# LuchnikovI/Differentiable-quantum-circuit-cuda

Hardware: AMD Instinct MI355X
Metric: gate-applications/sec (fwd+bwd) at n qubits (higher is better)
Workload: dtype c64 (f32)

## Files before the change

differentiable-quantum-circuit-cuda_amd/csrc/qdc.hip:

```cpp
#include "qdc_circuit.hpp"
#include "qdc_primitives.hpp"
#include "qdc_spec.hpp"

namespace {
template <int R>
struct SpecCheckTwo {
  __device__ __forceinline__ void operator()(qdc::cx (&xf)[R], qdc::cx (&xb)[R], const qdc::SpecEnv& E) const {
    constexpr uint32_t z[32] = {};
    qdc::spec_xchg_imm<6, false>(xf, E, z, z);
    qdc::spec_xchg<6, false>(xb, E, z, z, z, z);
  }
};
template <int R, int TB>
struct SpecCheckOne {
  __device__ __forceinline__ void operator()(qdc::cx (&x)[R], const qdc::SpecEnv& E) const {
    constexpr uint32_t z[32] = {};
    qdc::spec_xchg_imm<TB, true>(x, E, z, z);
    qdc::spec_xchg<TB, true>(x, E, z, z, z, z);
  }
};
}
#define QDC_SPEC_CHECK(name, threads, pass)                                                       \
  __global__ __launch_bounds__(threads) void name(qdc::chunk* f, qdc::chunk* b, const qdc::fop* ops, \
                                                  const qdc::cx* mats, qdc::fgeo fg, uint32_t l0,    \
// ... 354 lines not shown
    }
    x.prof.on = on != 0;
  }
  return nullptr;
}

QDC_API size_t qdc_circuit_profile_collect(qdc_circuit* c, qdc_kernel_stat* out, size_t cap) {
  std::vector<qdc::Ctx*> xs;
  for (auto& d : c->impl.devs) xs.push_back(&d->ctx);
  return qdc::prof_collect(xs, out, cap);
}

QDC_API size_t qdc_circuit_host_times(qdc_circuit* c, double* out, size_t n, int reset) {
  size_t k = 0;
  for (int d = 0; d < 2; ++d)
    for (int j = 0; j < 6; ++j, ++k)
      if (out && k < n) out[k] = c->impl.host_ms[d][j];
  if (reset)
    for (auto& row : c->impl.host_ms)
      for (double& v : row) v = 0;
  return std::min<size_t>(n, 12);
}

QDC_API const char* qdc_build_info(void) {
#ifdef QDC_F64
  return "qdc f64 gfx950";
#else
  return "qdc f32 gfx950";
#endif
}

QDC_API size_t qdc_fusion_schedule(size_t local_qubits, int backward, size_t first_inject,
                                   const int* kinds, const unsigned char* inexact,
                                   size_t n_instr, const qdc_plan_op* plan, size_t n_plan,
                                   int lcmin, int max_ops, unsigned* item_info, size_t item_cap,
                                   unsigned* stage_len, size_t stage_cap, unsigned* op_order,
                                   size_t op_cap) {
  std::vector<qdc::Instr> ins(n_instr);
  for (size_t k = 0; k < n_instr; ++k) ins[k] = qdc::Instr{kinds[k], 0, 0};
  std::vector<uint8_t> sens(n_instr, 0);
  if (inexact)
    for (size_t k = 0; k < n_instr; ++k) sens[k] = inexact[k] ? 1 : 0;
  qdc::FusionPlanner P{ins, sens, (uint32_t)local_qubits, true, true,
                             max_ops > 0 ? (uint32_t)std::min(max_ops, qdc::FMAX_OPS)
                                         : (uint32_t)qdc::FMAX_OPS,
                             lcmin > 0 ? (uint32_t)lcmin : 3u};
  using qdc::Knob;
  P.tile2_chunks = qdc::knob_uint(Knob::TILE2_CHUNKS, P.tile2_chunks);
  P.tile1_chunks = qdc::knob_uint(Knob::TILE1_CHUNKS, P.tile1_chunks);
  P.permute = P.rq_grad = qdc::knob_int(Knob::SCHED_RQ, 0) != 0;
  P.permute = qdc::knob_int(Knob::SCHED_PERM, P.permute) != 0;
  P.mirror = qdc::knob_int(Knob::SCHED_MIRROR, P.mirror) != 0;
  P.defer_q1 = qdc::knob_int(Knob::DEFER_Q1, P.defer_q1) != 0;
  P.perm_low = qdc::knob_uint(Knob::RQ_PERM_LOW, P.perm_low);
  P.gamma_stage_cap = qdc::knob_int(Knob::RQ_GSTAGE, P.gamma_stage_cap) != 0;
  P.split_dens = qdc::knob_int(Knob::DENS_SPLIT, P.split_dens) != 0;
  std::vector<qdc_plan_op> pl(plan, plan + n_plan);
  const std::vector<qdc::FusionItem> items = P.fuse_items(pl, backward != 0, first_inject);
  size_t ns = 0, no = 0;
  for (size_t i = 0; i < items.size(); ++i) {
    const qdc::FusionItem& it = items[i];
    std::vector<std::vector<uint32_t>> stages;
    if (it.type == 2)
      stages = P.stage_partition(it.ops, pl, backward != 0);
    else
      stages.push_back(it.ops);
    if (i >= item_cap || ns + stages.size() > stage_cap) return SIZE_MAX;
    unsigned* info = item_info + 12 * i;
    info[0] = (unsigned)it.type;
    info[1] = (unsigned)stages.size();
    info[2] = it.lc;
    info[3] = it.h;
    for (int k = 0; k < 8; ++k) info[4 + k] = k < (int)qdc::FMAX_ROWS ? it.hb[k] : 0u;
    for (const auto& st : stages) {
      stage_len[ns++] = (unsigned)st.size();
      for (uint32_t op : st) {
        if (no >= op_cap) return SIZE_MAX;
        op_order[no++] = op;
      }
    }
  }
  return items.size();
}

QDC_API int qdc_gate_plan(unsigned n, unsigned R, unsigned pos2, unsigned pos1,
                          int two_states, int far_tile, unsigned* out) {
  if (!out || (R != 2 && R != 4) || n < 2 || n > 62 || pos2 >= n || pos1 >= n ||
      (R == 2 && pos2 != pos1) || (R == 4 && pos2 == pos1))
    return -1;
  const qdc::Plan p = qdc::plan_gate(n, (int)R, pos2, pos1, two_states != 0, 1024u, far_tile != 0);
  const uint64_t cnt = p.tile ? p.tg.ntiles : p.g.items;
  const unsigned v[10] = {p.tile ? 1u : 0u, (unsigned)p.mode, p.tg.l, p.tg.h, p.tg.hb0, p.tg.hb1,
                          p.tg.t1, p.tg.t2, (unsigned)(cnt & 0xffffffffu), (unsigned)(cnt >> 32)};
  for (int i = 0; i < 10; ++i) out[i] = v[i];
  return 0;
}

QDC_API int qdc_lane_plan(unsigned n, unsigned R, unsigned pos2, unsigned pos1, int reduces,
                          unsigned* out) {
  if (!out || (R != 2 && R != 4) || n < 2 || n > 62 || pos2 >= n || pos1 >= n ||
      (R == 2 && pos2 != pos1) || (R == 4 && pos2 == pos1))
    return -1;
  qdc::Plan p;
  if (!qdc::plan_lane(n, (int)R, pos2, pos1, 2048u, (reduces & 1) != 0, p, 1, (reduces & 2) ? 10u : 6u))
    return 1;
  const qdc::lgeo& g = p.lg;
// ... 305 lines not shown
```

differentiable-quantum-circuit-cuda_amd/csrc/qdc_circuit.hpp:

```cpp
#pragma once

#include <algorithm>
#include <cstring>
#include <memory>
#include <vector>

#include <rccl/rccl.h>

#include "qdc/circuit.h"
#include "qdc_device.hpp"
#include "qdc_shard.hpp"
#include "qdc_stage.hpp"
#include "qdc_fusion.hpp"
#include "qdc_jit.hpp"

namespace qdc {

struct Flat {
  const qdc_complex* data;
  std::vector<size_t> off;
  std::vector<size_t> len;
  Flat(const qdc_complex* d, const size_t* lens, size_t n) : data(d), off(n), len(n) {
    size_t o = 0;
    for (size_t i = 0; i < n; ++i) {
// ... 162 lines not shown
    return nullptr;
  }
  void destroy() {
    for (auto e : ev) (void)hipEventDestroy(e);
    ev.clear();
    for (auto c : comms) (void)ncclCommDestroy(c);
    comms.clear();
  }
};

struct Circuit {
  uint32_t n = 0;
  uint32_t g = 0;
  uint32_t nl = 0;
  uint32_t gap_bits = 0;
  uint64_t gm = 0;
  std::vector<std::unique_ptr<DevRes>> devs;
  Exchange ex;
  std::vector<Shard> sh;
  QubitMap layout;
  size_t dens_cap = 0, grads_cap = 0;
  cx* host_out = nullptr;
  size_t host_cap = 0;
  std::vector<Instr> ins;
  struct Knobs {
    int fuse = 1;
    uint32_t fuse_max_ops = FMAX_OPS;
    uint32_t fuse_lcmin = 3;
    int fuse_meas = 1;
    int use_rq = 1;
    int rq_stats = 0;
    RqKnobs rqk;
    int rq64 = 1;
    int rq_order = 2;
    int spec_mode = 1;
    uint32_t spec_min_qubits = 22;
    uint32_t spec_max = 160;
    int spec_fwd = 1;
    int spec_async = sizeof(real) == 4 ? 1 : 0;
    int rq_permute = 1;
    int rq_perm_shard = 1;
    int rq_grad32 = 1;
    int rq_maxcl = 1;
    uint32_t rq_perm_low = 0;
    int rq_gstage = 1;
    uint32_t tile1_chunks = FusionPlanner::TILE_CHUNKS_1;
    int diag_inject = 1;
    int early_inject = 1;
    int dens1_kernel = 1;
    int dens_split = 1;
    int mirror = 1;
    int spec_half = 1;
    int defer_q1 = 1;
    uint32_t fused_blocks = 0;
    int sched_cache_on = 1;
    int state_ilv = 1;
    uint32_t state_ilv_bits = 12;

    template <class K, class F>
    static void each(K& k, F&& f) {
      f(Knob::FUSE, k.fuse);
      f(Knob::FUSE_MAX_OPS, k.fuse_max_ops, 1, FMAX_OPS);
      f(Knob::FUSE_MEAS, k.fuse_meas);
      f(Knob::FUSE_LCMIN, k.fuse_lcmin, 1, LOWBITS);
      f(Knob::FUSED_BLOCKS, k.fused_blocks, 1, (int)NBMAX);
      f(Knob::RQ, k.use_rq);
      f(Knob::RQ64, k.rq64);
      f(Knob::RQ_STATS, k.rq_stats);
      f(Knob::RW, k.rqk.rq_wave);
      f(Knob::RQ_PF, k.rqk.rq_prefetch);
      f(Knob::RQ_SLOTS5, k.rqk.rq_slots5);
      f(Knob::RQ_ORDER, k.rq_order);
      f(Knob::RQ_PERM, k.rq_permute);
      f(Knob::RQ_PERM_SHARD, k.rq_perm_shard);
      f(Knob::RQ_PERM_LOW, k.rq_perm_low);
      f(Knob::RQ_GRAD32, k.rq_grad32);
      f(Knob::RQ_MAXCL, k.rq_maxcl);
      f(Knob::RQ_GSTAGE, k.rq_gstage);
      f(Knob::TILE1_CHUNKS, k.tile1_chunks);
      f(Knob::DIAG_INJECT, k.diag_inject);
      f(Knob::EARLY_INJECT, k.early_inject);
      f(Knob::DENS1, k.dens1_kernel);
      f(Knob::DENS_SPLIT, k.dens_split);
      f(Knob::MIRROR, k.mirror);
      f(Knob::DEFER_Q1, k.defer_q1);
      f(Knob::SCHED_CACHE, k.sched_cache_on);
      f(Knob::SPEC, k.spec_mode);
      f(Knob::SPEC_MIN_QUBITS, k.spec_min_qubits);
      f(Knob::SPEC_MAX, k.spec_max);
      f(Knob::SPEC_FWD, k.spec_fwd);
      f(Knob::SPEC_ASYNC, k.spec_async);
      f(Knob::SPEC_HALF, k.spec_half);
      f(Knob::STATE_ILV, k.state_ilv);
      f(Knob::STATE_ILV_BITS, k.state_ilv_bits, 4, 24);
    }
    const char* read() {
      each(*this, KnobRead{});
      constexpr uint32_t T1 = FusionPlanner::TILE_CHUNKS_1, T2 = FusionPlanner::TILE_CHUNKS_2;
      if (tile1_chunks != T1 && tile1_chunks != T2)
        return fail("%s must be %u or %u", KNOB_TABLE[(int)Knob::TILE1_CHUNKS].name, T1, T2);
      return nullptr;
    }
  } k;
  double host_ms[2][6] = {};
  using hclock = std::chrono::steady_clock;
  static double ms_between(hclock::time_point a, hclock::time_point b) {
    return std::chrono::duration<double, std::milli>(b - a).count();
  }
  void host_record(int dir, const hclock::time_point (&t)[6]) {
    host_ms[dir][0] += 1;
    for (int k = 1; k < 6; ++k) host_ms[dir][k] += ms_between(t[k - 1], t[k]);
  }
  std::map<std::vector<uint32_t>, SpecEntry> spec_cache;
  uint64_t spec_epoch = 0;
  bool mirror_on() const {
    return k.mirror && k.fuse && k.fuse_max_ops >= 2 && k.use_rq && (sizeof(real) == 4 || k.rq64);
  }
  const char* rq_variant(bool two, uint32_t tbits, const RqVariant*& V) const {
    V = rq_select(two, tbits, k.rqk, mirror_on());
    if (!V)
      return fail("no register-resident kernel for a %u-amplitude %s tile", 1u << tbits,
                  two ? "two-state" : "one-state");
    return nullptr;
  }
  bool rq_keep(const RqVariant& V) const { return k.spec_half && V.ns == 5; }

  bool dry = false;
  std::vector<unsigned char> dry_prog;
  std::vector<SpecEntry*> dry_specs;
  struct TraceOp {
    uint32_t dir, item, q2, q1, R, diag, mirrored, single;
    qdc_complex m[16];
  };
  bool tracing = false;
  std::vector<TraceOp> trace;
  size_t trace_from = 0;
  std::vector<uint8_t> inexact;
  std::vector<std::pair<const void*, uint32_t>> fused_resident_cache;
// ... 428 lines not shown
      size_t ng = f.stages.size();
      while (ng > 0 && is_meas(mrec.plan[f.stages[ng - 1][0]])) --ng;
      for (size_t j = ng; j < f.stages.size(); ++j)
        for (uint32_t fi : f.stages[j])
          if (!is_meas(mrec.plan[fi])) return false;
      if (ng < f.stages.size()) {
        Item m = shell();
        for (size_t j = f.stages.size(); j-- > ng;) {
          const uint32_t bi = push(f.stages[j][0]);
          m.ops.push_back(bi);
          m.stages.push_back({bi});
        }
        if (m.ops.size() == 1) {
          m.type = 0;
          m.stages.clear();
        }
        items.push_back(std::move(m));
      }
      if (ng == 0) continue;
      Item b = shell();
      for (auto it = f.swaps.rbegin(); it != f.swaps.rend(); ++it) b.swaps.push_back(*it);
      for (size_t j = ng; j-- > 0;) {
        std::vector<uint32_t> st;
        for (size_t t = f.stages[j].size(); t-- > 0;) {
          if (is_meas(mrec.plan[f.stages[j][t]])) return false;
          const uint32_t bi = push(f.stages[j][t]);
          st.push_back(bi);
          b.ops.push_back(bi);
        }
        b.stages.push_back(std::move(st));
        b.mirror_of.push_back({(uint32_t)k, (uint32_t)j});
      }
      items.push_back(std::move(b));
    }
    first_inject = first_injection(pl);
    return true;
  }
  size_t first_injection(const std::vector<qdc_plan_op>& pl) const {
    for (size_t i = 0; i < pl.size(); ++i)
      if (pl[i].type == QDC_PLAN_OP && is_diff_density(ins[pl[i].instr].kind)) return i;
    return pl.size();
  }
  static constexpr uint32_t TILE_CHUNKS_1 = FusionPlanner::TILE_CHUNKS_1;
  static constexpr uint32_t TILE_CHUNKS_2 = FusionPlanner::TILE_CHUNKS_2;
  FusionPlanner planner() const {
    FusionPlanner P{ins, inexact, nl, k.fuse != 0, k.fuse_meas != 0, k.fuse_max_ops, k.fuse_lcmin};
    P.permute = k.rq_permute && k.use_rq && (g == 0 || k.rq_perm_shard) && sizeof(real) == 4;
    P.ng = g;
    P.rq_grad = k.rq_grad32 && k.use_rq && (sizeof(real) == 4 || k.rq64);
    if (k.rq_perm_low) P.perm_low = k.rq_perm_low;
    P.tile1_chunks = k.tile1_chunks;
    P.mirror = mirror_on() && sched_mirror;
    P.defer_q1 = k.defer_q1 != 0;
    P.gamma_stage_cap = k.rq_gstage != 0;
    P.split_dens = k.dens_split != 0;
    return P;
  }
  bool is_meas(const qdc_plan_op& op) const { return planner().is_meas(op); }
  std::vector<Item> fuse_items(std::vector<qdc_plan_op>& plan, bool backward,
                               size_t first_inject = SIZE_MAX) const {
    std::vector<Item> items;
    for (FusionItem& f : planner().fuse_items(plan, backward, first_inject)) {
      Item it;
      static_cast<FusionItem&>(it) = std::move(f);
      if (it.type == 2) it.stages = planner().stage_partition(it.ops, plan, backward);
      items.push_back(std::move(it));
    }
    return items;
  }
  struct SchedCache {
    bool valid = false;
    size_t first_inject = 0;
    bool mirror = false;
    std::vector<qdc_plan_op> in_plan, out_plan;
    std::vector<uint8_t> inexact;
    std::vector<Item> items;
  };
  SchedCache sched_cache[2];
  bool sched_mirror = false;
  static bool same_plan(const std::vector<qdc_plan_op>& a, const std::vector<qdc_plan_op>& b) {
    if (a.size() != b.size()) return false;
    for (size_t i = 0; i < a.size(); ++i) {
      const qdc_plan_op &x = a[i], &y = b[i];
      if (x.type != y.type || x.instr != y.instr || x.pos2 != y.pos2 || x.pos1 != y.pos1 ||
          x.nvictims != y.nvictims || x.pack != y.pack)
        return false;
      for (unsigned k = 0; k < x.nvictims && k < 8; ++k)
        if (x.victims[k] != y.victims[k]) return false;
    }
    return true;
  }
  std::vector<Item> schedule(std::vector<qdc_plan_op>& plan, bool backward, size_t first_inject) {
    SchedCache& c = sched_cache[backward ? 1 : 0];
    if (k.sched_cache_on && c.valid && c.first_inject == first_inject && c.inexact == inexact &&
        c.mirror == sched_mirror && same_plan(c.in_plan, plan)) {
      plan = c.out_plan;
      return c.items;
    }
    c.valid = false;
    c.in_plan = plan;
    std::vector<Item> items = fuse_items(plan, backward, first_inject);
    if (k.sched_cache_on) {
      c.out_plan = plan;
      c.items = items;
      c.inexact = inexact;
      c.first_inject = first_inject;
// ... 1036 lines not shown
```

differentiable-quantum-circuit-cuda_amd/csrc/qdc_fusion.hpp:

```cpp
#pragma once

#include <stdint.h>

#include <algorithm>
#include <vector>

#include "qdc/circuit.h"
#include "qdc_kernels.hpp"
#include "qdc_knobs.hpp"
#include "qdc_rq.hpp"
#include "qdc_shard.hpp"

namespace qdc {

struct Instr {
  int kind;
  uint32_t a;
  uint32_t b;
};

inline bool is_q1_gate(int k) {
  return k == QDC_CONST_Q1 || k == QDC_CONST_Q1_NONU || k == QDC_VAR_Q1 || k == QDC_VAR_Q1_NONU;
}
inline bool is_q2_dense(int k) {
  return k == QDC_CONST_Q2 || k == QDC_VAR_Q2 || k == QDC_CONST_Q2_NONU || k == QDC_VAR_Q2_NONU;
}
inline bool is_diag(int k) { return k == QDC_CONST_Q2_DIAG || k == QDC_VAR_Q2_DIAG; }
inline bool is_const(int k) {
  return k == QDC_CONST_Q1 || k == QDC_CONST_Q1_NONU || k == QDC_CONST_Q2 ||
         k == QDC_CONST_Q2_NONU || k == QDC_CONST_Q2_DIAG;
}
inline bool is_var(int k) {
  return k == QDC_VAR_Q1 || k == QDC_VAR_Q1_NONU || k == QDC_VAR_Q2 || k == QDC_VAR_Q2_NONU ||
         k == QDC_VAR_Q2_DIAG;
}
inline bool is_nonu(int k) {
  return k == QDC_CONST_Q1_NONU || k == QDC_VAR_Q1_NONU || k == QDC_CONST_Q2_NONU ||
         k == QDC_VAR_Q2_NONU;
}
inline bool is_density(int k) {
  return k == QDC_Q1_DENSITY || k == QDC_Q2_DENSITY || k == QDC_DIFF_Q1_DENSITY ||
         k == QDC_DIFF_Q2_DENSITY;
}
inline bool is_diff_density(int k) {
  return k == QDC_DIFF_Q1_DENSITY || k == QDC_DIFF_Q2_DENSITY;
}
inline bool is_q1_density(int k) { return k == QDC_Q1_DENSITY || k == QDC_DIFF_Q1_DENSITY; }
inline int gate_len(int k) { return is_q2_dense(k) ? 16 : 4; }

struct FusionItem {
  int type;
  std::vector<uint32_t> ops;
  uint32_t lc = 0, h = 0, hb[FMAX_ROWS] = {};
  std::vector<std::pair<uint32_t, uint32_t>> swaps;
};

struct FusionPlanner {
  static constexpr uint32_t TILE_CHUNKS_1 = 2048;
  static constexpr uint32_t TILE_CHUNKS_2 = 1024;
  const std::vector<Instr>& ins;
  const std::vector<uint8_t>& inexact;
  uint32_t nl;
  bool fuse;
  bool fuse_meas;
  uint32_t fuse_max_ops;
  uint32_t fuse_lcmin;
  uint32_t tile2_chunks = TILE_CHUNKS_2;
  uint32_t tile1_chunks = TILE_CHUNKS_1;
  bool permute = false;
  bool rq_grad = false;
  bool gamma_stage_cap = true;
  uint32_t perm_low = (uint32_t)LV + 3;
  uint32_t ng = 0;
  bool mirror = false;
  bool defer_q1 = true;
  bool split_dens = true;

  static uint32_t log2_of(uint64_t x) {
    uint32_t k = 0;
    while ((1ull << k) < x) ++k;
    return k;
  }

  uint64_t chunk_bits_of(uint32_t p) const { return p >= (uint32_t)LV ? 1ull << (p - LV) : 0ull; }
  bool tile_config(uint64_t mask, uint32_t T, uint32_t& lc, uint32_t& h, uint32_t* hb) const {
    const uint32_t cbits = nl - LV;
    if (cbits < T) return false;
    for (int l = (int)T; l >= (int)fuse_lcmin; --l) {
      uint32_t rows = 0, tmp[64];
      for (uint32_t c = (uint32_t)l; c < cbits; ++c)
        if (mask >> c & 1ull) tmp[rows++] = c;
      if (rows > (uint32_t)FMAX_ROWS || (uint32_t)l + rows > T) continue;
      for (uint32_t c = (uint32_t)l; c < cbits && (uint32_t)l + rows < T; ++c)
        if (!(mask >> c & 1ull)) tmp[rows++] = c;
      if ((uint32_t)l + rows != T || rows > (uint32_t)FMAX_ROWS) continue;
      std::sort(tmp, tmp + rows);
      lc = (uint32_t)l;
      h = rows;
      for (uint32_t k = 0; k < rows; ++k) hb[k] = tmp[k];
      return true;
    }
    return false;
  }
  bool tile_fits(uint64_t mask, uint32_t T) const {
    if (nl - LV < T) return false;
    for (int l = (int)T; l >= (int)fuse_lcmin; --l) {
      const uint32_t rows = (uint32_t)__builtin_popcountll(mask >> l);
      if (rows <= (uint32_t)FMAX_ROWS && (uint32_t)l + rows <= T) return true;
    }
    return false;
  }

  bool is_meas(const qdc_plan_op& op) const {
    return op.type == QDC_PLAN_OP && is_density(ins[op.instr].kind);
  }
  uint32_t op_class(const qdc_plan_op& op, bool backward) const {
    if (op.type != QDC_PLAN_OP) return 0;
    const bool inex = op.instr < inexact.size() && inexact[op.instr];
    if (mirror && !backward)
      return order_class(ins[op.instr].kind, false, inex) | order_class(ins[op.instr].kind, true, inex);
    return order_class(ins[op.instr].kind, backward, inex);
  }
  static uint32_t conflicts_of(uint32_t c) { return order_conflicts(c); }
  bool is_gate_op(const qdc_plan_op& op) const {
    if (op.type != QDC_PLAN_OP) return false;
    const int k = ins[op.instr].kind;
    return is_const(k) || is_var(k);
  }
  uint64_t op_bits(const qdc_plan_op& op) const {
// ... 77 lines not shown
    remap_map(nv, mn);
    for (uint32_t p = 0; p < nl + ng; ++p) mvi[mv[p]] = p;
    for (uint32_t x = 0; x < nl + ng; ++x) out[x] = mn[pi[mvi[x]]];
    pi.swap(out);
    r.pack = 0;
    for (uint32_t j = 0; j < ng; ++j) {
      r.victims[j] = nv[j];
      r.pack |= (nv[j] != nl - ng + j) ? 1 : 0;
    }
  }

  std::vector<FusionItem> fuse_items(std::vector<qdc_plan_op>& plan, bool backward,
                                     size_t first_inject = SIZE_MAX) const {
    std::vector<FusionItem> items;
    const bool mfwd = mirror && !backward;
    const uint32_t T = log2_of((backward || mfwd) ? tile2_chunks : tile1_chunks);
    const bool on = fuse && fuse_max_ops >= 2;
    size_t msplit = SIZE_MAX;
    if (mfwd)
      for (size_t k = plan.size(); k-- > 0;)
        if (plan[k].type == QDC_PLAN_OP && is_meas(plan[k]) &&
            (ins[plan[k].instr].kind == QDC_DIFF_Q1_DENSITY ||
             ins[plan[k].instr].kind == QDC_DIFF_Q2_DENSITY)) {
          msplit = k + 1;
          break;
        }
    auto fusable = [&](size_t k) {
      const qdc_plan_op& op = plan[k];
      if (!(is_gate_op(op) || (fuse_meas && is_meas(op))) || !tile_fits(op_bits(op), T))
        return false;
      return !(backward && is_meas(op) && k < first_inject);
    };
    size_t i = 0;
    while (i < plan.size()) {
      const qdc_plan_op& op = plan[i];
      if (op.type == QDC_PLAN_REMAP) {
        items.push_back(FusionItem{1, {(uint32_t)i}});
        ++i;
        continue;
      }
      if (!on || !fusable(i)) {
        items.push_back(FusionItem{0, {(uint32_t)i}});
        ++i;
        continue;
      }
      size_t j = i;
      while (j < plan.size() && plan[j].type == QDC_PLAN_OP && fusable(j) &&
             !(backward && j == first_inject && j > i) && !(j == msplit && j > i))
        ++j;
      const bool two = (backward && i >= first_inject) || mfwd;
      const bool gstage = two && rq_grad && gamma_stage_cap;
      const uint32_t gmax = gstage ? fuse_max_ops
                            : (two && rq_grad) ? (uint32_t)FMAX_GRAD_RQ : (uint32_t)FMAX_GRAD;
      std::vector<uint32_t> rem;
      for (size_t k = i; k < j; ++k) rem.push_back((uint32_t)k);
      while (!rem.empty()) {
        uint64_t mask = 0, blocked = 0;
        uint32_t nred = 0;
        uint32_t ndens = 0;
        uint32_t left = 0;
        std::vector<uint32_t> pass, rest;
        int kind = -1;
        for (uint32_t k : rem) {
          const qdc_plan_op& g = plan[k];
          const uint64_t q = (1ull << g.pos2) | (1ull << g.pos1);
          const bool meas = is_meas(g);
          const uint32_t cls = op_class(g, backward);
          const uint32_t isred = mfwd ? (is_var(ins[g.instr].kind) ? 1u : 0u)
                                 : ((!backward && meas) || (two && is_var(ins[g.instr].kind))) ? 1u : 0u;
          if ((backward && kind >= 0 && (int)meas != kind) || (mfwd && kind == 1 && !meas) ||
              (!backward && split_dens && kind == 0 && meas) ||
              (q & blocked) ||
              (mfwd && meas && ndens + 1 > (uint32_t)FMAX_GRAD) ||
              (conflicts_of(cls) & left) || pass.size() >= fuse_max_ops ||
              nred + isred > gmax || !tile_fits(mask | op_bits(g), T)) {
            blocked |= q;
            left |= cls;
            rest.push_back(k);
            continue;
          }
          pass.push_back(k);
          mask |= op_bits(g);
          nred += isred;
          ndens += (mfwd && meas) ? 1u : 0u;
          kind = (int)meas;
        }
        if (gstage && nred > (uint32_t)FMAX_GRAD_RQ) {
          bool cut = false;
          while (pass.size() > 1 && gamma_stages(pass, plan, !mfwd) > (uint32_t)FMAX_GRAD_RQ) {
            rest.push_back(pass.back());
            pass.pop_back();
            cut = true;
          }
          if (cut) {
            std::sort(rest.begin(), rest.end());
            mask = 0;
            for (uint32_t k : pass) mask |= op_bits(plan[k]);
          }
        }
        if (defer_q1 && defer_trailing_q1(pass, rest, plan, backward)) {
          mask = 0;
          for (uint32_t k : pass) mask |= op_bits(plan[k]);
        }
        if (pass.size() == 1) {
          items.push_back(FusionItem{0, pass});
        } else {
          FusionItem it{2, pass};
          tile_config(mask, T, it.lc, it.h, it.hb);
          bool gates_only = it.lc >= NLOW - LV;
          for (uint32_t k : pass) gates_only = gates_only && is_gate_op(plan[k]);
          if (permute && gates_only) permute_after(it, plan, rest, j);
          items.push_back(it);
        }
        rem.swap(rest);
      }
      i = j;
    }
    return items;
  }

  bool defer_trailing_q1(std::vector<uint32_t>& pass, std::vector<uint32_t>& rest,
                         const std::vector<qdc_plan_op>& plan, bool backward) const {
    if (pass.size() < 2 || rest.empty()) return false;
    const std::vector<std::vector<uint32_t>> sts = stage_partition(pass, plan, backward);
    if (sts.size() < 2) return false;
    std::vector<uint32_t> moved;
    size_t kept_stages = sts.size();
    for (const auto& st : sts) {
      if (kept_stages <= 1) break;
      bool q1only = true;
      for (uint32_t k : st)
        q1only = q1only && is_gate_op(plan[k]) && plan[k].pos2 == plan[k].pos1 &&
                 plan[k].pos2 == plan[st[0]].pos2;
      if (!q1only) continue;
      const uint32_t qb = plan[st[0]].pos2;
      const uint64_t qm = 1ull << qb;
      bool free = true;
      for (uint32_t x : st) {
        const uint32_t cx = op_class(plan[x], backward);
        for (uint32_t y : pass) {
          if (y <= x || std::find(st.begin(), st.end(), y) != st.end()) continue;
          if (std::find(moved.begin(), moved.end(), y) != moved.end()) continue;
          const uint64_t yq = (1ull << plan[y].pos2) | (1ull << plan[y].pos1);
          if ((yq & qm) || (conflicts_of(cx) & op_class(plan[y], backward))) free = false;
        }
      }
      if (!free) continue;
      const qdc_plan_op* next = nullptr;
      for (uint32_t k : rest)
        if (k > st.back() && (((1ull << plan[k].pos2) | (1ull << plan[k].pos1)) & qm)) {
          next = &plan[k];
          break;
        }
      if (!next || !is_gate_op(*next) || next->pos2 == next->pos1) continue;
      moved.insert(moved.end(), st.begin(), st.end());
      --kept_stages;
    }
    if (moved.empty()) return false;
    std::vector<uint32_t> keep;
    for (uint32_t k : pass)
      if (std::find(moved.begin(), moved.end(), k) == moved.end()) keep.push_back(k);
    pass.swap(keep);
    rest.insert(rest.end(), moved.begin(), moved.end());
    std::sort(rest.begin(), rest.end());
    return true;
  }

  uint32_t gamma_stages(const std::vector<uint32_t>& pass, const std::vector<qdc_plan_op>& plan,
                        bool backward = true) const {
    uint32_t n = 0;
    for (const auto& st : stage_partition(pass, plan, backward)) {
      bool var = false;
      for (uint32_t k : st) var = var || (plan[k].type == QDC_PLAN_OP && is_var(ins[plan[k].instr].kind));
      n += var ? 1u : 0u;
    }
    return n;
  }

  std::vector<std::vector<uint32_t>> stage_partition(const std::vector<uint32_t>& pass,
                                                     const std::vector<qdc_plan_op>& plan,
                                                     bool backward) const {
    std::vector<std::vector<uint32_t>> stages;
    std::vector<uint32_t> rem = pass;
    while (!rem.empty()) {
      std::vector<uint32_t> st, rest;
      uint64_t q = 0, blocked = 0;
      uint32_t left = 0;
      bool closed = false;
      for (uint32_t k : rem) {
        if (closed) {
          rest.push_back(k);
          continue;
        }
        const qdc_plan_op& g = plan[k];
        const uint64_t gq = (1ull << g.pos2) | (1ull << g.pos1);
        const bool meas = is_meas(g);
        const uint32_t cls = op_class(g, backward);
        bool bad = (gq & blocked) || (conflicts_of(cls) & left);
        if (!bad && meas) {
          if (st.empty()) {
            st.push_back(k);
            closed = true;
            continue;
          }
          bad = true;
        }
        if (!bad && __builtin_popcountll(q | gq) > 2) bad = true;
        if (bad) {
          blocked |= gq;
          left |= cls;
          rest.push_back(k);
          continue;
        }
        st.push_back(k);
        q |= gq;
      }
      stages.push_back(std::move(st));
      rem.swap(rest);
    }
    return stages;
  }

};

struct RqStage {
  uint32_t kind, t1, t2;
  uint64_t deps = 0;
};
constexpr int RQ_SLOTS_MAX = 5;
struct RqLayout {
  uint32_t ns = 4;
  uint32_t slot[RQ_SLOTS_MAX] = {~0u, ~0u, ~0u, ~0u, ~0u};
  bool tfix = false;
  uint32_t tfirst[3] = {0, 0, 0};
  static RqLayout empty(uint32_t ns) {
    RqLayout L;
    L.ns = ns;
    return L;
  }
  bool operator==(const RqLayout& o) const {
    if (ns != o.ns || tfix != o.tfix) return false;
    for (uint32_t s = 0; s < ns; ++s)
      if (slot[s] != o.slot[s]) return false;
    return !tfix || (tfirst[0] == o.tfirst[0] && tfirst[1] == o.tfirst[1] &&
                     tfirst[2] == o.tfirst[2]);
  }
  uint32_t threads(uint32_t T, uint32_t* out) const {
    uint32_t k = 0;
    if (tfix)
      for (int i = 0; i < 3; ++i) out[k++] = tfirst[i];
    for (uint32_t q = 0; q < T && k < 8; ++q) {
      if (holds(q)) continue;
      if (tfix && (q == tfirst[0] || q == tfirst[1] || q == tfirst[2])) continue;
      out[k++] = q;
    }
    return k;
  }
  int find(uint32_t q) const {
    for (uint32_t s = 0; s < ns; ++s)
      if (slot[s] == q) return (int)s;
// ... 256 lines not shown
```

differentiable-quantum-circuit-cuda_amd/csrc/qdc_knobs.hpp:

```cpp
#pragma once

#include <stdint.h>

#include <algorithm>
#include <climits>
#include <cstdio>
#include <cstdlib>
#include <string>

namespace qdc {

enum class KnobScope { Process, Context, Circuit, Call, Hook };

#define QDC_KNOBS(X)                                                                               \
                                                        \
  X(DYN, Context, "35",                                                                            \
    "static share (% of the fair share) of a dynamic-tail pass; 100: static only")                 \
  X(DYN_GRAN, Context, "1",                                                                        \
    "smallest granule (tiles per grab, a power of two <= 32) of a reducing dynamic tail")          \
  X(EVENT_FENCE, Context, "0",                                                                     \
    "1: the profiler's HIP events are default events (system-scope fence per record)")             \
  X(GRID_CAP, Context, "1048576", "grid cap of the single-gate streaming kernels")                 \
  X(RED_CAP, Context, "2048", "grid of the single-gate reduction kernels (<= 4096)")               \
  X(REV_RED, Context, "4096",                                                                      \
// ... 7 lines not shown
  X(TILE2_WIDE, Context, "2", "two-state tile-family launches on 2^(9 + w)-chunk tiles")           \
  X(TILE1_WIDE, Context, "2", "one-state tile-family launches on 2^(10 + w)-chunk tiles")          \
  X(LANE, Context, "2",                                                                            \
    "single-gate ops on the LANE family, bits: 1 reverse, 2 streaming one-state, 4 densities "     \
    "/ gradients")                                                                                 \
  X(DIAG_RU, Context, "16",                                                                        \
    "chunks per state in flight per thread of the diagonal reverse kernels")                       \
  X(DIAG_Q, Context, "1", "0: diagonal reverse launches on k_diag instead of k_diag_q")            \
  X(DIAG_RED, Context, "4096", "grid of the diagonal reverse's reducing launches (<= 4096)")       \
  X(TILE_PF, Context, "1", "0: tile-family blocks of several tiles do not prefetch the next tile") \
  X(LANE_BLK, Context, "1",                                                                        \
    "0: far-target streaming LANE launches stay on the wave variant, not k_lane_blk")              \
  X(LANE_TILE_BITS, Context, "0x8800000",                                                          \
    "mask of target byte strides 2^b whose one-state q1 applications run on the tile family")      \
  X(LANE_NOBLK_BITS, Context, "0x808000",                                                          \
    "mask of target byte strides 2^b whose far LANE applications run on the wave variant")         \
  X(LANE_U, Context, "8,1,4",                                                                      \
    "units in flight per wave of LANE launches, \"u0,u1,u2\" per op class as QDC_LANE")            \
                                                   \
  X(FUSE, Circuit, "1", "0: one HBM pass per gate (single-gate kernels only)")                     \
  X(FUSE_MAX_OPS, Circuit, "32", "gates per fused pass (1 .. FMAX_OPS)")                           \
  X(FUSE_MEAS, Circuit, "1", "0: densities / cotangent injections stay single passes")             \
  X(FUSE_LCMIN, Circuit, "3", "minimum contiguous chunk bits of a fused tile (1 .. 6)")            \
  X(FUSED_BLOCKS, Circuit, "0",                                                                    \
    "grid of fused passes (1 .. 4096); 0: as many blocks as are resident")                         \
  X(RQ, Circuit, "1", "0: gate passes on the LDS-tile kernel, not the register-resident ones")     \
  X(RQ64, Circuit, "1", "0: f64 gate passes stay on the LDS-tile kernel")                          \
  X(RQ_STATS, Circuit, "0",                                                                        \
    "1: print each register-resident pass's counts to stderr; 2: its stages too")                  \
  X(RW, Circuit, "1", "register-resident kernel choice, a bit mask (qdc_variant.hpp)")             \
  X(RQ_PF, Circuit, "1", "0: one-state register-resident passes do not prefetch the next tile")    \
  X(RQ_SLOTS5, Circuit, "1", "0: f32 one-wave passes plan four register slots, not five")          \
  X(RQ_ORDER, Circuit, "2",                                                                        \
    "register-resident tile order: 0 block-contiguous, 1 grid-strided, 2 XCD-aware")               \
  X(RQ_PERM, Circuit, "1", "0: gate-only passes keep the qubit layout (no in-store permutation)")  \
  X(RQ_PERM_SHARD, Circuit, "1", "0: no permuting passes on sharded circuits")                     \
  X(RQ_PERM_LOW, Circuit, "0", "low positions a permuting pass fills; 0: the planner's default")   \
  X(RQ_GRAD32, Circuit, "1",                                                                       \
    "0: two-state passes hold FMAX_GRAD instead of FMAX_GRAD_RQ Gamma stages")                     \
  X(RQ_MAXCL, Circuit, "1", "0: relayouts chosen greedily instead of by max closure")              \
  X(RQ_GSTAGE, Circuit, "1",                                                                       \
    "0: two-state passes capped by variable gates instead of Gamma stages")                        \
  X(TILE1_CHUNKS, Circuit, "2048", "one-state fused tile in chunks: 2048 or 1024")                 \
  X(DIAG_INJECT, Circuit, "1",                                                                     \
    "0: runs of diagonal cotangent injections stay fused injection passes")                        \
  X(EARLY_INJECT, Circuit, "1",                                                                    \
    "0: the backward's leading diagonal injection waits for its program")                          \
  X(DENS1, Circuit, "1", "0: read-only one-qubit density passes on k_fused instead of k_dens1")    \
  X(DENS_SPLIT, Circuit, "1", "0: a forward pass may hold gates and densities together")           \
  X(MIRROR, Circuit, "1",                                                                          \
    "mirrored reverse sweeps; 0: the backward schedules itself; 2: failing to mirror is an "       \
    "error")                                                                                       \
  X(DEFER_Q1, Circuit, "1", "0: trailing one-qubit stages of a pass stay there")                   \
  X(SCHED_CACHE, Circuit, "1",                                                                     \
    "0: schedule every call instead of reusing the last call's schedule")                          \
  X(SPEC, Circuit, "1",                                                                            \
    "specialized passes: 0 off, 1 from QDC_SPEC_MIN_QUBITS local qubits, 2 always")                \
  X(SPEC_MIN_QUBITS, Circuit, "22", "local qubits from which QDC_SPEC=1 specializes")              \
  X(SPEC_MAX, Circuit, "160", "distinct specialized kernels a call compiles in line")              \
  X(SPEC_FWD, Circuit, "1", "0: only the two-state reverse passes are specialized")                \
  X(SPEC_ASYNC, Circuit, "f32: 1, f64: 0",                                                         \
    "programs above QDC_SPEC_MAX compile in the background; 0: they stay generic")                 \
  X(SPEC_HALF, Circuit, "1",                                                                       \
    "0: five-slot specialized passes relayout through the full LDS buffer")                        \
  X(STATE_ILV, Circuit, "1", "0: separate fwd / bwd allocations instead of the interleaved pair")  \
  X(STATE_ILV_BITS, Circuit, "12", "block size of the interleaved pair, 2^b chunks (4 .. 24)")     \
                                                                   \
  X(SPEC_IMM, Process, "0", "1: specialized relayouts address LDS by immediate offsets")           \
  X(RQ_SWZ, Process, "1", "0: register-resident relayouts use the k_fused LDS swizzle")            \
  X(PACK_TILE, Process, "1", "0: remap packing on the direct kernel instead of LDS tiles")         \
  X(JIT_DIR, Process, "$XDG_CACHE_HOME/qdc_jit, $HOME/.cache/qdc_jit or /tmp/qdc_jit_<uid>",       \
    "code-object cache of the specialized kernels")                                                \
  X(JIT_PREBUILT, Process, "<lib>/../jit-prebuilt",                                                \
    "directory of kernels compiled ahead of time; 0: none")                                        \
  X(SRC_DIR, Process, "<lib>/../csrc", "kernel headers the specialized passes compile against")    \
  X(HIPCC, Process, "$ROCM_PATH/bin/hipcc", "compiler of the specialized passes")                  \
                                                                         \
  X(JIT_JOBS, Call, "min(hardware threads, 16) / ranks", "parallel hipcc processes (<= 16)")       \
  X(JIT_ASYNC_JOBS, Call, "as QDC_JIT_JOBS", "kernels per batch of the background compiler")       \
  X(JIT_WAIT_S, Call, "900", "seconds to wait for a kernel another process compiles")              \
  X(JIT_KEEP, Call, "0", "1: keep the sources and logs of successful compiles")                    \
  X(QK_PAIR, Call, "1", "dense k-qubit kernel: 0 no paired 16-B accesses, 2 paired at k = 4 too")  \
  X(QK_WIDE, Call, "k >= 4: 1, else 0",                                                            \
    "dense k-qubit kernel: doubled batches per wave iteration")                                    \
  X(QK_PF, Call, "k = 3: 2, k = 5: 1, else 0",                                                     \
    "dense k-qubit kernel: 1 software-pipelined batches, 2 doubled too")                           \
  X(QK_GRID, Call, "4096", "block cap of the dense k-qubit kernels' grids")                        \
  X(QK_LDS, Call, "k = 3: 2, else 1",                                                              \
    "low targets from which a dense gate runs as LDS-staged tiles; 0: never")                      \
  X(QKL_VAR, Call, "1", "k_qkl variant: 0 not pipelined, 1 pipelined, 2 half the tiles at k = 5")  \
  X(QKG_GRID, Call, "resident blocks", "block cap of the dense gradient / density kernel")         \
  X(PAULI_GRID, Call, "per kernel", "block cap of the Pauli-sum kernels")                          \
                                                     \
  X(SCHED_RQ, Hook, "0",                                                                           \
    "qdc_fusion_schedule: permuting passes and the register-resident Gamma cap")                   \
  X(SCHED_PERM, Hook, "as QDC_SCHED_RQ", "qdc_fusion_schedule: permuting passes alone")            \
  X(SCHED_MIRROR, Hook, "0", "qdc_fusion_schedule: the mirrored forward schedule")                 \
  X(TILE2_CHUNKS, Hook, "1024", "qdc_fusion_schedule: two-state fused tile in chunks")             \
  X(RQ_KEEP, Hook, "0", "qdc_rq_plan: every relayout keeps a register slot (half buffers)")        \
  X(PRECOMPILE_DUMP, Hook, "unset",                                                                \
    "qdc_precompile: directory that receives each kernel's source")                                \
  X(PRECOMPILE_COUNT, Hook, "0", "qdc_precompile: 1 counts the kernels without compiling them")

enum class Knob : int {
#define QDC_KNOB_ID(id, scope, dflt, effect) id,
  QDC_KNOBS(QDC_KNOB_ID)
// ... 78 lines not shown
```

Before: 4787.

## Search fused-pass qubit tiles greedily to maximize stages per pass

Replaces the first-come greedy pass scan in the fusion planner with a seeded greedy search over candidate tile qubit sets. Each candidate is scored by how many stages it packs, keeping the best when it beats the baseline scan. Also lets trailing one-qubit stages be deferred per qubit, and stops stage partitioning from pairing two lone one-qubit gates that will not later form a two-qubit gate. The aim is fewer passes over the state vector, each doing more work. The cost is more host-side planning time, which is mitigated by the schedule cache.

New measurement: 5296 (median of 6 runs). +10.7%, better.

```diff
diff --git a/differentiable-quantum-circuit-cuda_amd/csrc/qdc.hip b/differentiable-quantum-circuit-cuda_amd/csrc/qdc.hip
--- a/differentiable-quantum-circuit-cuda_amd/csrc/qdc.hip
+++ b/differentiable-quantum-circuit-cuda_amd/csrc/qdc.hip
@@ -430,6 +430,7 @@
   P.permute = qdc::knob_int(Knob::SCHED_PERM, P.permute) != 0;
   P.mirror = qdc::knob_int(Knob::SCHED_MIRROR, P.mirror) != 0;
   P.defer_q1 = qdc::knob_int(Knob::DEFER_Q1, P.defer_q1) != 0;
+  P.search = qdc::knob_int(Knob::FUSE_SEARCH, P.search) != 0;
   P.perm_low = qdc::knob_uint(Knob::RQ_PERM_LOW, P.perm_low);
   P.gamma_stage_cap = qdc::knob_int(Knob::RQ_GSTAGE, P.gamma_stage_cap) != 0;
   P.split_dens = qdc::knob_int(Knob::DENS_SPLIT, P.split_dens) != 0;
diff --git a/differentiable-quantum-circuit-cuda_amd/csrc/qdc_circuit.hpp b/differentiable-quantum-circuit-cuda_amd/csrc/qdc_circuit.hpp
--- a/differentiable-quantum-circuit-cuda_amd/csrc/qdc_circuit.hpp
+++ b/differentiable-quantum-circuit-cuda_amd/csrc/qdc_circuit.hpp
@@ -238,6 +238,7 @@
     int mirror = 1;
     int spec_half = 1;
     int defer_q1 = 1;
+    int fuse_search = 1;
     uint32_t fused_blocks = 0;
     int sched_cache_on = 1;
     int state_ilv = 1;
@@ -270,6 +271,7 @@
       f(Knob::DENS_SPLIT, k.dens_split);
       f(Knob::MIRROR, k.mirror);
       f(Knob::DEFER_Q1, k.defer_q1);
+      f(Knob::FUSE_SEARCH, k.fuse_search);
       f(Knob::SCHED_CACHE, k.sched_cache_on);
       f(Knob::SPEC, k.spec_mode);
       f(Knob::SPEC_MIN_QUBITS, k.spec_min_qubits);
@@ -804,6 +806,7 @@
     P.tile1_chunks = k.tile1_chunks;
     P.mirror = mirror_on() && sched_mirror;
     P.defer_q1 = k.defer_q1 != 0;
+    P.search = k.fuse_search != 0;
     P.gamma_stage_cap = k.rq_gstage != 0;
     P.split_dens = k.dens_split != 0;
     return P;
diff --git a/differentiable-quantum-circuit-cuda_amd/csrc/qdc_fusion.hpp b/differentiable-quantum-circuit-cuda_amd/csrc/qdc_fusion.hpp
--- a/differentiable-quantum-circuit-cuda_amd/csrc/qdc_fusion.hpp
+++ b/differentiable-quantum-circuit-cuda_amd/csrc/qdc_fusion.hpp
@@ -75,6 +75,7 @@
   bool mirror = false;
   bool defer_q1 = true;
   bool split_dens = true;
+  bool search = true;
 
   static uint32_t log2_of(uint64_t x) {
     uint32_t k = 0;
@@ -258,75 +259,196 @@
       const bool gstage = two && rq_grad && gamma_stage_cap;
       const uint32_t gmax = gstage ? fuse_max_ops
                             : (two && rq_grad) ? (uint32_t)FMAX_GRAD_RQ : (uint32_t)FMAX_GRAD;
+      const PassRules rules{backward, mfwd, two, gstage, gmax, T};
       std::vector<uint32_t> rem;
       for (size_t k = i; k < j; ++k) rem.push_back((uint32_t)k);
       while (!rem.empty()) {
-        uint64_t mask = 0, blocked = 0;
-        uint32_t nred = 0;
-        uint32_t ndens = 0;
-        uint32_t left = 0;
-        std::vector<uint32_t> pass, rest;
-        int kind = -1;
-        for (uint32_t k : rem) {
-          const qdc_plan_op& g = plan[k];
-          const uint64_t q = (1ull << g.pos2) | (1ull << g.pos1);
-          const bool meas = is_meas(g);
-          const uint32_t cls = op_class(g, backward);
-          const uint32_t isred = mfwd ? (is_var(ins[g.instr].kind) ? 1u : 0u)
-                                 : ((!backward && meas) || (two && is_var(ins[g.instr].kind))) ? 1u : 0u;
-          if ((backward && kind >= 0 && (int)meas != kind) || (mfwd && kind == 1 && !meas) ||
-              (!backward && split_dens && kind == 0 && meas) ||
-              (q & blocked) ||
-              (mfwd && meas && ndens + 1 > (uint32_t)FMAX_GRAD) ||
-              (conflicts_of(cls) & left) || pass.size() >= fuse_max_ops ||
-              nred + isred > gmax || !tile_fits(mask | op_bits(g), T)) {
-            blocked |= q;
-            left |= cls;
-            rest.push_back(k);
-            continue;
+        ScannedPass sp = search ? search_pass(plan, rem, rules)
+                                : scan_pass(plan, rem.data(), rem.size(), rules, ~0ull, false);
+        if (sp.ops.size() == 1) {
+          items.push_back(FusionItem{0, sp.ops});
+        } else {
+          FusionItem it{2, sp.ops};
+          tile_config(sp.mask, T, it.lc, it.h, it.hb);
+          bool gates_only = it.lc >= NLOW - LV;
+          for (uint32_t k : sp.ops) gates_only = gates_only && is_gate_op(plan[k]);
+          if (permute && gates_only) permute_after(it, plan, sp.rest, j);
+          items.push_back(it);
+        }
+        rem.swap(sp.rest);
+      }
+      i = j;
+    }
+    return items;
+  }
+
+  struct PassRules {
+    bool backward, mfwd, two, gstage;
+    uint32_t gmax, T;
+  };
+  struct ScannedPass {
+    std::vector<uint32_t> ops, rest;
+    uint64_t mask = 0;
+  };
+  ScannedPass scan_pass(const std::vector<qdc_plan_op>& plan, const uint32_t* rem, size_t nrem,
+                        const PassRules& r, uint64_t allowed, bool per_qubit) const {
+    const bool backward = r.backward, mfwd = r.mfwd, two = r.two;
+    ScannedPass sp;
+    std::vector<uint32_t>& pass = sp.ops;
+    std::vector<uint32_t>& rest = sp.rest;
+    uint64_t mask = 0, blocked = 0;
+    uint32_t nred = 0;
+    uint32_t ndens = 0;
+    uint32_t left = 0;
+    int kind = -1;
+    for (size_t x = 0; x < nrem; ++x) {
+      if ((blocked & allowed) == allowed) {
+        rest.insert(rest.end(), rem + x, rem + nrem);
+        break;
+      }
+      const uint32_t k = rem[x];
+      const qdc_plan_op& g = plan[k];
+      const uint64_t q = (1ull << g.pos2) | (1ull << g.pos1);
+      const bool meas = is_meas(g);
+      const uint32_t cls = op_class(g, backward);
+      const uint32_t isred = mfwd ? (is_var(ins[g.instr].kind) ? 1u : 0u)
+                             : ((!backward && meas) || (two && is_var(ins[g.instr].kind))) ? 1u : 0u;
+      if ((q & ~allowed) ||
+          (backward && kind >= 0 && (int)meas != kind) || (mfwd && kind == 1 && !meas) ||
+          (!backward && split_dens && kind == 0 && meas) ||
+          (q & blocked) ||
+          (mfwd && meas && ndens + 1 > (uint32_t)FMAX_GRAD) ||
+          (conflicts_of(cls) & left) || pass.size() >= fuse_max_ops ||
+          nred + isred > r.gmax || !tile_fits(mask | op_bits(g), r.T)) {
+        blocked |= q;
+        left |= cls;
+        rest.push_back(k);
+        continue;
+      }
+      pass.push_back(k);
+      mask |= op_bits(g);
+      nred += isred;
+      ndens += (mfwd && meas) ? 1u : 0u;
+      kind = (int)meas;
+    }
+    if (r.gstage && nred > (uint32_t)FMAX_GRAD_RQ) {
+      bool cut = false;
+      while (pass.size() > 1 && gamma_stages(pass, plan, !mfwd) > (uint32_t)FMAX_GRAD_RQ) {
+        rest.push_back(pass.back());
+        pass.pop_back();
+        cut = true;
+      }
+      if (cut) std::sort(rest.begin(), rest.end());
+    }
+    if (defer_q1) defer_trailing_q1(pass, rest, plan, backward, per_qubit);
+    for (uint32_t k : pass) sp.mask |= op_bits(plan[k]);
+    return sp;
+  }
+
+  static constexpr size_t SEARCH_SEEDS = 8;
+  static constexpr size_t SEARCH_WINDOW = 512;
+
+  uint64_t tile_positions(uint64_t pos, uint32_t T) const {
+    uint32_t lc, h, hb[64];
+    if (!tile_config(pos >> LV, T, lc, h, hb)) return 0;
+    uint64_t a = (1ull << (LV + lc)) - 1;
+    for (uint32_t r = 0; r < h; ++r) a |= 1ull << (LV + hb[r]);
+    return a;
+  }
+  static uint64_t pos_bits(const qdc_plan_op& g) { return (1ull << g.pos2) | (1ull << g.pos1); }
+
+  ScannedPass search_pass(const std::vector<qdc_plan_op>& plan, const std::vector<uint32_t>& rem,
+                          const PassRules& r) const {
+    ScannedPass base = scan_pass(plan, rem.data(), rem.size(), r, ~0ull, false);
+    const size_t nw = std::min(rem.size(), SEARCH_WINDOW);
+    auto stages_of = [&](const ScannedPass& p) {
+      return (uint32_t)stage_partition(p.ops, plan, r.backward).size();
+    };
+    auto at_cap = [&](const ScannedPass& p, uint32_t st) {
+      return p.ops.size() >= fuse_max_ops || (r.gstage && st >= (uint32_t)FMAX_GRAD_RQ) ||
+             p.rest.empty();
+    };
+    auto width = [&](const ScannedPass& p) {
+      uint64_t q = (1ull << NLOW) - 1;
+      for (uint32_t k : p.ops) q |= pos_bits(plan[k]);
+      return (uint32_t)__builtin_popcountll(q);
+    };
+    const uint32_t base_st = stages_of(base);
+    if (at_cap(base, base_st) || nw < 3) return base;
+
+    struct Cand {
+      uint64_t tile;
+      ScannedPass p;
+      uint32_t st;
+    };
+    std::vector<Cand> cands;
+    auto eval = [&](uint64_t tile) -> size_t {
+      for (size_t c = 0; c < cands.size(); ++c)
+        if (cands[c].tile == tile) return c;
+      Cand c{tile, scan_pass(plan, rem.data(), nw, r, tile, true), 0};
+      c.st = stages_of(c.p);
+      cands.push_back(std::move(c));
+      return cands.size() - 1;
+    };
+    uint64_t seen = 0;
+    size_t seeds = 0;
+    for (size_t x = 0; x < nw && seeds < SEARCH_SEEDS; ++x) {
+      const uint64_t sq = pos_bits(plan[rem[x]]);
+      const bool ready = !(sq & seen);
+      seen |= sq;
+      if (!ready) continue;
+      ++seeds;
+      uint64_t want = sq | ((1ull << NLOW) - 1);
+      uint64_t tile = tile_positions(want, r.T);
+      while (tile) {
+        const size_t cur = eval(tile);
+        const uint32_t cur_st = cands[cur].st;
+        if (at_cap(cands[cur].p, cur_st)) break;
+        const std::vector<uint32_t> rest = cands[cur].p.rest;
+        uint64_t handled = 0, best_add = 0, best_tile = 0;
+        int64_t best_gain = 0, best_cost = 0;
+        for (uint32_t k : rest) {
+          const uint64_t q = pos_bits(plan[k]);
+          const uint64_t first = q & tile & ~handled;
+          handled |= q & tile;
+          const uint64_t add = q & ~tile;
+          if (!first || !add) continue;
+          const uint64_t t2 = tile_positions(want | q, r.T);
+          if (!t2 || t2 == tile) continue;
+          const int64_t gain = (int64_t)cands[eval(t2)].st - (int64_t)cur_st;
+          const int64_t cost = __builtin_popcountll(add);
+          if (!best_tile || gain * best_cost > best_gain * cost) {
+            best_gain = gain;
+            best_cost = cost;
+            best_add = q;
+            best_tile = t2;
           }
-          pass.push_back(k);
-          mask |= op_bits(g);
-          nred += isred;
-          ndens += (mfwd && meas) ? 1u : 0u;
-          kind = (int)meas;
-        }
-        if (gstage && nred > (uint32_t)FMAX_GRAD_RQ) {
-          bool cut = false;
-          while (pass.size() > 1 && gamma_stages(pass, plan, !mfwd) > (uint32_t)FMAX_GRAD_RQ) {
-            rest.push_back(pass.back());
-            pass.pop_back();
-            cut = true;
-          }
-          if (cut) {
-            std::sort(rest.begin(), rest.end());
-            mask = 0;
-            for (uint32_t k : pass) mask |= op_bits(plan[k]);
-          }
-        }
-        if (defer_q1 && defer_trailing_q1(pass, rest, plan, backward)) {
-          mask = 0;
-          for (uint32_t k : pass) mask |= op_bits(plan[k]);
-        }
-        if (pass.size() == 1) {
-          items.push_back(FusionItem{0, pass});
-        } else {
-          FusionItem it{2, pass};
-          tile_config(mask, T, it.lc, it.h, it.hb);
-          bool gates_only = it.lc >= NLOW - LV;
-          for (uint32_t k : pass) gates_only = gates_only && is_gate_op(plan[k]);
-          if (permute && gates_only) permute_after(it, plan, rest, j);
-          items.push_back(it);
-        }
-        rem.swap(rest);
-      }
-      i = j;
-    }
-    return items;
+          if ((handled & tile) == tile) break;
+        }
+        if (!best_tile) break;
+        want |= best_add;
+        tile = best_tile;
+      }
+    }
+    size_t best = cands.size();
+    uint32_t best_st = base_st, best_w = 0;
+    for (size_t c = 0; c < cands.size(); ++c) {
+      if (cands[c].st <= best_st && best == cands.size()) continue;
+      const uint32_t w = width(cands[c].p);
+      if (best == cands.size() || cands[c].st > best_st || (cands[c].st == best_st && w < best_w)) {
+        best = c;
+        best_st = cands[c].st;
+        best_w = w;
+      }
+    }
+    if (best == cands.size()) return base;
+    ScannedPass chosen = scan_pass(plan, rem.data(), rem.size(), r, cands[best].tile, true);
+    return stages_of(chosen) > base_st ? chosen : base;
   }
 
   bool defer_trailing_q1(std::vector<uint32_t>& pass, std::vector<uint32_t>& rest,
-                         const std::vector<qdc_plan_op>& plan, bool backward) const {
+                         const std::vector<qdc_plan_op>& plan, bool backward,
+                         bool per_qubit = false) const {
     if (pass.size() < 2 || rest.empty()) return false;
     const std::vector<std::vector<uint32_t>> sts = stage_partition(pass, plan, backward);
     if (sts.size() < 2) return false;
@@ -337,30 +459,38 @@
       bool q1only = true;
       for (uint32_t k : st)
         q1only = q1only && is_gate_op(plan[k]) && plan[k].pos2 == plan[k].pos1 &&
-                 plan[k].pos2 == plan[st[0]].pos2;
+                 (per_qubit || plan[k].pos2 == plan[st[0]].pos2);
       if (!q1only) continue;
-      const uint32_t qb = plan[st[0]].pos2;
-      const uint64_t qm = 1ull << qb;
-      bool free = true;
-      for (uint32_t x : st) {
-        const uint32_t cx = op_class(plan[x], backward);
-        for (uint32_t y : pass) {
-          if (y <= x || std::find(st.begin(), st.end(), y) != st.end()) continue;
-          if (std::find(moved.begin(), moved.end(), y) != moved.end()) continue;
-          const uint64_t yq = (1ull << plan[y].pos2) | (1ull << plan[y].pos1);
-          if ((yq & qm) || (conflicts_of(cx) & op_class(plan[y], backward))) free = false;
-        }
-      }
-      if (!free) continue;
-      const qdc_plan_op* next = nullptr;
-      for (uint32_t k : rest)
-        if (k > st.back() && (((1ull << plan[k].pos2) | (1ull << plan[k].pos1)) & qm)) {
-          next = &plan[k];
-          break;
-        }
-      if (!next || !is_gate_op(*next) || next->pos2 == next->pos1) continue;
-      moved.insert(moved.end(), st.begin(), st.end());
-      --kept_stages;
+      size_t gone = 0;
+      for (uint32_t qb : {plan[st.front()].pos2, plan[st.back()].pos2}) {
+        std::vector<uint32_t> grp;
+        for (uint32_t k : st)
+          if (plan[k].pos2 == qb && std::find(moved.begin(), moved.end(), k) == moved.end())
+            grp.push_back(k);
+        if (grp.empty()) continue;
+        const uint64_t qm = 1ull << qb;
+        bool free = true;
+        for (uint32_t x : grp) {
+          const uint32_t cx = op_class(plan[x], backward);
+          for (uint32_t y : pass) {
+            if (y <= x || std::find(grp.begin(), grp.end(), y) != grp.end()) continue;
+            if (std::find(moved.begin(), moved.end(), y) != moved.end()) continue;
+            const uint64_t yq = (1ull << plan[y].pos2) | (1ull << plan[y].pos1);
+            if ((yq & qm) || (conflicts_of(cx) & op_class(plan[y], backward))) free = false;
+          }
+        }
+        if (!free) continue;
+        const qdc_plan_op* next = nullptr;
+        for (uint32_t k : rest)
+          if (k > grp.back() && (((1ull << plan[k].pos2) | (1ull << plan[k].pos1)) & qm)) {
+            next = &plan[k];
+            break;
+          }
+        if (!next || !is_gate_op(*next) || next->pos2 == next->pos1) continue;
+        moved.insert(moved.end(), grp.begin(), grp.end());
+        gone += grp.size();
+      }
+      if (gone == st.size()) --kept_stages;
     }
     if (moved.empty()) return false;
     std::vector<uint32_t> keep;
@@ -393,7 +523,16 @@
       uint64_t q = 0, blocked = 0;
       uint32_t left = 0;
       bool closed = false;
-      for (uint32_t k : rem) {
+      auto pairs_up = [&](size_t x, uint64_t both) {
+        for (size_t y = x + 1; y < rem.size(); ++y) {
+          const qdc_plan_op& n = plan[rem[y]];
+          const uint64_t nq = (1ull << n.pos2) | (1ull << n.pos1);
+          if (nq & both) return nq == both && is_gate_op(n);
+        }
+        return true;
+      };
+      for (size_t x = 0; x < rem.size(); ++x) {
+        const uint32_t k = rem[x];
         if (closed) {
           rest.push_back(k);
           continue;
@@ -412,6 +551,9 @@
           bad = true;
         }
         if (!bad && __builtin_popcountll(q | gq) > 2) bad = true;
+        if (!bad && search && q && !(q & gq) && __builtin_popcountll(q) == 1 &&
+            __builtin_popcountll(gq) == 1 && !pairs_up(x, q | gq))
+          bad = true;
         if (bad) {
           blocked |= gq;
           left |= cls;
diff --git a/differentiable-quantum-circuit-cuda_amd/csrc/qdc_knobs.hpp b/differentiable-quantum-circuit-cuda_amd/csrc/qdc_knobs.hpp
--- a/differentiable-quantum-circuit-cuda_amd/csrc/qdc_knobs.hpp
+++ b/differentiable-quantum-circuit-cuda_amd/csrc/qdc_knobs.hpp
@@ -83,6 +83,8 @@
     "mirrored reverse sweeps; 0: the backward schedules itself; 2: failing to mirror is an "       \
     "error")                                                                                       \
   X(DEFER_Q1, Circuit, "1", "0: trailing one-qubit stages of a pass stay there")                   \
+  X(FUSE_SEARCH, Circuit, "1",                                                                     \
+    "0: a pass's qubits are whatever the scan meets first, not chosen by search")                  \
   X(SCHED_CACHE, Circuit, "1",                                                                     \
     "0: schedule every call instead of reusing the last call's schedule")                          \
   X(SPEC, Circuit, "1",                                                                            \
```
